# chalharu/rust-compression

Measured on AMD Instinct MI355X. Metric: BZip2 level-9 encode MB/s (input bytes, HBM-resident in and out: the kernels' rate; value_end_to_end is host buffer to host buffer at the C ABI), higher is better.
Workload: dtype u8/u32

## Files before the change

### rust-compression_amd/csrc/bzgpu.h

```cpp
#pragma once
#include <hip/hip_runtime.h>
#include <stdint.h>
#include <stddef.h>

namespace bzgpu {

typedef uint8_t u8;
typedef uint16_t u16;
typedef uint32_t u32;
typedef uint64_t u64;
typedef int64_t i64;

constexpr u32 kWave = 64;
constexpr u32 kMaxBlockLen = 900000;
constexpr u32 kSortTile = 8192;
constexpr u32 kSortThreads = 512;
constexpr u32 kTilesPerBlock = 110;
constexpr u32 kSlot = kTilesPerBlock * kSortTile;
constexpr u32 kPtSlot = kSlot / 8u * 10u;
constexpr u32 kPairWords = 65536u / 32u;
constexpr u32 kMaxBins = 2048;
constexpr u32 kPerK = 8;
constexpr u32 kGSize = 50;
constexpr u32 kMaxSelectors = 18002;
// ... 164 lines not shown
typedef u32 u32x4_t __attribute__((ext_vector_type(4)));
__device__ __forceinline__ void st_sc1_x4(u32 *p, uint4 v)
{
    const u32x4_t r = {v.x, v.y, v.z, v.w};
    asm volatile("global_store_dwordx4 %0, %1, off\n\ts_nop 1" : : "v"(p), "v"(r) : "memory");
}
__device__ __forceinline__ uint4 ld_sc1_x4(const u32 *p)
{
    u32x4_t r;
    asm volatile("global_load_dwordx4 %0, %1, off nt\n\ts_waitcnt vmcnt(0)" : "=v"(r) : "v"(p) : "memory");
    return make_uint4(r.x, r.y, r.z, r.w);
}

__device__ __forceinline__ void ld_sc1_x4_issue(const u32 *p, u32x4_t &r)
{
    asm volatile("global_load_dwordx4 %0, %1, off nt" : "=&v"(r) : "v"(p) : "memory");
}
__device__ __forceinline__ void ld_x4_wait_all() { asm volatile("s_waitcnt vmcnt(0)" : : : "memory"); }

constexpr u32 kCrcPoly = 0x04C11DB7u;

__host__ __device__ inline u32 gf_mulmod(u32 a, u32 b)
{
    u32 r = 0;
#pragma unroll 4
    for (int i = 31; i >= 0; --i) {
        r = (r << 1) ^ ((r & 0x80000000u) ? kCrcPoly : 0u);
        if ((b >> i) & 1u) r ^= a;
    }
    return r;
}

__device__ __forceinline__ u32 gf_xpow_bytes(u64 nbytes, const u32 *__restrict__ xp2)
{
    u32 r = 1u;
    for (u32 k = 0; nbytes; ++k, nbytes >>= 1)
        if (nbytes & 1u) r = gf_mulmod(r, xp2[k]);
    return r;
}

__device__ __forceinline__ u32 crc_bytes_raw(const u8 *__restrict__ p, u64 len, const u32 *s_tab)
{
    u32 crc = 0;
    for (u64 i = 0; i < len; ++i) crc = s_tab[(crc >> 24) ^ p[i]] ^ (crc << 8);
    return crc;
}


struct RleBuffers {
    i64 *tile_last;
    i64 *carry_in;
    u32 *tile_crc;
    u32 *tile_count;
    u16 *sub_off;
    i64 *sub_rs;
    u64 *tile_off;
    u64 *total;
    u64 *cut_result;
    u64 *scan_part;
    u32 *lb_ctl;
    u64 *lb_rs;
    u64 *lb_off;
};

struct CutPlan {
    u64 L;
    u64 g_base;
    u64 own_hi;
    u64 w_min;
    u64 j_lo, j_hi;
    u64 tb, t1;
    u64 t_last;
    u64 t_eval;
};
struct CutBuffers {
    u64 *step_t0;
    u32 *step_nt;
    u64 *step_w0;
    u32 *tab;
    u16 *comp;
};

struct BwtArgs {
    const u8 *rle;
    const BlockDesc *blocks;
    u32 nb;
    u32 tiles;
    u32 *SA, *R, *KA, *VA, *KB, *VB;
    u32 *tile_hist;
    u32 *bin_base;
    u32 *count;
    u32 *count2;
    u32 *tile_nf;
    u8 *flags;
    u64 *newbits;
    int *tile_last_old;
    int *tile_last_new;
    u32 *nonfinal;
    unsigned long long *active;
    u32 *maxnf;
    u32 *per_k, *per_shift;
    u32 *lin_p, *lin_sig;
    u32 *bin_cursor;
    u32 *pb_gate;
    u32 *loc_stats;
    u8 *L;
    u32 *orig_ptr;
    u8 *ptext;
    u32 *pair_bits;
    const u8 *sym_code;
    const u8 *keyinfo;
    u32 *gh_tiles;
    u32 *gbase;
    u32 pack_blocks;
    u64 *abits;
    u32 *tile_state;
    u32 *tickets;
    u32 *sort_err;
    u32 *epoch;
    u8 *per_aux;
    u32 per_keyshift;
    u32 per_wide;
    u32 per_links;
    u32 *fused_state;
    u32 *tile_state_all;
    u32 fused;
    size_t tile_state_bytes;
};
constexpr u32 kSortEpochs = 1024;

constexpr u32 kMtfStride = kSlot + 64;
struct MtfArgs {
    const BlockDesc *blocks;
    u32 nb;
    u32 tiles;
    const u8 *L;
    u32 heads;
    u32 dense_permille;
    u8 *H;
    u16 *headbits;
    u32 *hcount;
    u32 *tile_hcnt;
    u32 *tile_hbase;
    const u32 *inuse_bits;
    u8 *summ;
    u16 *summ_len;
    u8 *init_state;
    u8 *rank8;
    int *ztile_last;
    u32 *ztile_cnt;
    u32 *zstate;
    u32 *ztick;
    u32 fused_zle;
    u16 *mtf;
    u32 *mtf_freq;
    BlockOut *out;
};

constexpr u32 kLim = 17;
constexpr u32 kLmRow = 2 * kMaxAlpha + 4;
constexpr u32 kLmWords = 2 * kLim * kLmRow + 5 * kMaxAlpha + 64;
constexpr u32 kSelStride = kMaxSelectors + 14;
constexpr u32 kGboStride = kMaxSelectors + 2;
struct HuffArgs {
    const BlockDesc *blocks;
    u32 nb;
    const u16 *mtf;
    u32 mtf_stride;
    const u32 *mtf_freq;
    const u32 *inuse_bits;
    const u32 *crc;
    const u32 *orig_ptr;
    u8 *selector;
    u32 *code_len;
    u32 *group_bitoff;
    u32 *lm_scratch;
    u8 *glen;
    unsigned long long *pack;
    u32 *rfreq;
    u32 *hlm;
    u32 *pass_stats;
    u32 *stream;
    BlockOut *out;
    u32 *error_flag;
};

struct AsmBlock {
    u64 src_word;
    u64 bit_len;
    u64 dst_bit;
};
struct PackBlock {
    u64 src_word, dst_word, nwords;
};
struct RleBatchItem {
    u64 in_off;
    u64 len;
    u64 rle_off;
};
struct FrameItem {
    u64 first_word;
    u64 trailer_bit;
    u32 combined_crc;
    u32 pad;
};

constexpr int BZ_DEC_E_DATA = -1;
struct DecCand {
    u64 bitpos;
    u32 type;
    u32 pad;
};
struct DecBlockInfo {
    u64 end_bit;
    u32 status;
    u32 stored_crc;
    u32 orig_ptr;
    u32 randomised;
    u32 n_in_use;
    u32 nsym;
    u32 next_head;
    u32 next_bits;
    u8 seq2unseq[256];
};

constexpr u32 kDecSampleStep = 128;
constexpr u32 kDecSamples = kMaxBlockLen / kDecSampleStep + 3;
constexpr u32 kSegCap = 4 * kDecSampleStep;
constexpr u32 kDecSubs = kSlot / 64;
struct KernelProf;
struct DecArgs {
    u32 nb;
    u32 tiles, sub_wgs;
    u32 cw;
    const u32 *slot;
    const DecBlockInfo *info;
    const u16 *sym;
    const u32 *nblock_max;
    u8 *perm;
    u32 *chunk_emit;
    u32 *tt_len;
    u32 *err;
    u8 *L;
    u32 *T;
    u8 *X;
    u32 *samp_next, *samp_len, *samp_off;
    u32 *cycle_len;
    uint4 *sub_trans;
    u32 *sub_off;
    u8 *sub_state;
    u32 *work_ctr;
    uint4 *walk_meta;
    u8 *seg_buf;
    u32 *seg_cont;
    u32 *long_list;
    u32 *out_len;
    u32 *thist;
    u32 *tbase;
    u32 *crc;
};
void launch_dec_scan(hipStream_t st, const u8 *in, u64 nbytes, DecCand *cands, u32 cap, u32 *count);
void launch_dec_blocks(hipStream_t st, const u8 *in, u64 nbytes, const DecCand *cands, u32 ncand, DecBlockInfo *info,
                       u16 *sym, u8 *sel_scratch);
constexpr u32 kDecEntrySkip = 0xFFFFFFFFu;
struct DecEntry {
    u64 off, len;
    u32 first_cand, ncand;
};
enum : u32 { kChainOk = 0, kChainData = 1, kChainMagicFirst = 2, kChainMagic = 3 };
struct DecChainEntry {
    u32 verdict;
    u32 streams;
    u32 irregular;
    u32 ntrue;
};
struct DecChainCand {
    u32 is_true, max_len;
    u32 stored_crc, nsym;
};
void launch_dec_scan_batch(hipStream_t st, const u8 *in, u64 span0, u64 span_end, const DecEntry *ents, u32 nent,
                           DecCand *cands, u32 cap, u32 *count);
void launch_dec_blocks_batch(hipStream_t st, const u8 *in, const DecEntry *ents, const DecCand *cands, u32 ncand,
                             DecBlockInfo *info, u16 *sym, u8 *sel_scratch);
void launch_dec_chain_batch(hipStream_t st, const u8 *in, const DecEntry *ents, u32 e0, u32 ne, const DecCand *cands,
                            u32 cand0, const DecBlockInfo *info, DecChainEntry *out_ent, DecChainCand *out_cand);
void launch_dec_mtf(hipStream_t st, const DecArgs &a, KernelProf *prof, int *rec);
void launch_dec_gather_windows(hipStream_t st, const u8 *in, u64 nbytes, const u64 *bases, u32 nw, u8 *out);
void launch_dec_walks(hipStream_t st, const DecArgs &a, u32 walk_wgs, hipStream_t st2, hipEvent_t ev_a, hipEvent_t ev_b,
                      KernelProf *prof, int rec[4]);
void launch_dec_expand(hipStream_t st, const DecArgs &a, const u64 *out_base, u8 *out);
void launch_dec_crc(hipStream_t st, const DecArgs &a, const u64 *out_base, const u8 *out, u32 max_out_len,
                    const u32 *crc_tab, const u32 *xp2, const u32 *xp16);

enum KernelId {
    KID_RADIX_HIST = 0,
    KID_RADIX_SCAN,
    KID_RADIX_SCATTER,
    KID_GROUP_FLAGS,
    KID_GROUP_APPLY,
    KID_LAST_COLUMN,
    KID_RADIX_SCATTER_LB,
    KID_GHIST_TEXT,
    KID_GHIST_SCAN,
    KID_RANK_PLACE,
    KID_PHASE_B_LOCAL,
    KID_GROUP_REFINE,
// ... 82 lines not shown
```

### rust-compression_amd/csrc/engine.hip

```cpp
#include "engine_state.h"

#include <algorithm>
#include <chrono>
#include <cstdio>
#include <cstdlib>
#include <cstring>
#include <vector>

#define MAILCHK(st, ...)                                                             \
    do {                                                                             \
        const MailSeg mail_segs_[] = {__VA_ARGS__};                                  \
        if (mail_fetch((st), mail_segs_, (int)(sizeof(mail_segs_) / sizeof(mail_segs_[0]))) != 0) return BZ_E_UNEXPECTED; \
    } while (0)

static int span_begin(bz_gpu_engine *g, int stage, hipStream_t st = nullptr)
{
    bz_gpu_engine::Span s;
    s.stage = stage;
    s.st = st ? st : g->st;
    if (hipEventCreate(&s.a) != hipSuccess || hipEventCreate(&s.b) != hipSuccess) return -1;
    (void)hipEventRecord(s.a, s.st);
    g->spans.push_back(s);
    return (int)g->spans.size() - 1;
}
// ... 600 lines not shown
        *j_next = j0 + closed;
        return BZ_OK;
    }
    ++g->cut_stats[0];
    if (res[0] > max_blocks) return BZ_E_UNEXPECTED;
    sc.tb = std::min<u64>(start_in / kRleTile, t0);
    sc.start_in = start_in;
    sc.nb = (size_t)res[0];
    sc.pending = true;
    sc.image_done = true;
    sc.span = -1;
    *n_blocks = sc.nb;
    *next_in = sc.nb || is_last ? res[1] : start_in;
    *s_next = res[3];
    *j_next = res[4];
    sp.want_halo_total = D;
    return BZ_OK;
}
static int slab_spec_finish(bz_gpu_engine *g, SlabSpec &sp, SlabCuts &sc)
{
    if (!sc.pending) return BZ_OK;
    if (!sp.image_done) return slab_image(g, sc);
    const RleBuffers rb = rle_buffers(g);
    const u64 t0 = g->slab_t0;
    sc.span = span_begin(g, 0);
    g->h_halo_total = sp.want_halo_total;
    if (sc.tb < t0) {
        launch_rle_scan(g->st, g->d_in, g->n_in, sc.tb, t0, sc.start_in, g->crc_tab.as<u32>(), g->xp16.as<u32>(), rb);
        launch_rle_count(g->st, g->d_in, g->n_in, sc.tb, t0, sc.start_in, -1, rb, nullptr);
        launch_rle_prefix(g->st, sc.tb, t0, rb, false);
        HIPCHK(hipMemcpyAsync(&g->h_halo_total, rb.total, 8, hipMemcpyDeviceToHost, g->st));
        image_launch(g, g->st, sc.tb, t0, sc.start_in, rb, g->rle.as<u8>() + sp.halo_cap - sp.want_halo_total);
    }
    HIPCHK(hipStreamWaitEvent(g->st, g->ev_aux, 0));
    return slab_image(g, sc);
}

extern "C" int bz_gpu_partition_slab_finish(bz_gpu_engine *g, uint64_t start_in, int is_last, size_t *n_blocks,
                                            uint64_t *next_in, int *tail_block)
{
    if (!g) return BZ_E_PARAM;
    SlabCuts sc;
    const int rc = slab_cuts(g, start_in, is_last, true, sc, n_blocks, next_in, tail_block);
    if (rc != BZ_OK) {
        if (sc.span >= 0) { span_end(g, sc.span); spans_collect(g); }
        return rc;
    }
    return slab_image(g, sc);
}

extern "C" int bz_gpu_partition(bz_gpu_engine *g, int level, const void *d_in, size_t n, int mode,
                                size_t *n_blocks, size_t *consumed, int *tail_block)
{
    if (!g || level < 1 || level > 9) return BZ_E_PARAM;
    if (n_blocks) *n_blocks = 0;
    if (consumed) *consumed = 0;
    if (tail_block) *tail_block = 0;
    const u64 ntiles = (n + kRleTile - 1) / kRleTile;
    int64_t last = -1;
    int rc = bz_gpu_partition_slab_begin(g, level, d_in, n, 0, ntiles, &last);
    if (rc != BZ_OK || n == 0) return rc;
    if ((rc = bz_gpu_partition_slab_count(g, -1)) != BZ_OK) return rc;
    uint64_t next = 0;
    rc = bz_gpu_partition_slab_finish(g, 0, mode == BZ_ACTION_RUN ? 0 : 1, n_blocks, &next, tail_block);
    if (consumed) *consumed = (size_t)next;
    return rc;
}

static BwtArgs make_bwt_args(bz_gpu_engine *g, u32 nb)
{
    BwtArgs x;
    x.rle = g->rle.as<u8>();
    x.blocks = g->lblocks.as<BlockDesc>();
    x.nb = nb;
    x.tiles = kTilesPerBlock;
    x.SA = g->SA.as<u32>();
    x.R = g->R.as<u32>();
    x.KA = g->KA.as<u32>();
    x.VA = g->VA.as<u32>();
    x.KB = g->KB.as<u32>();
    x.VB = g->VB.as<u32>();
    x.tile_hist = g->tile_hist.as<u32>();
    x.count = g->count.as<u32>();
    x.count2 = g->count2.as<u32>();
    x.tile_nf = g->tile_nf.as<u32>();
    x.bin_base = g->bin_base.as<u32>();
    x.flags = g->flags.as<u8>();
    x.newbits = g->newbits.as<u64>();
    x.tile_last_old = g->tlo.as<int>();
    x.tile_last_new = g->tln.as<int>();
    x.nonfinal = g->nonfinal.as<u32>();
    x.active = g->active.as<unsigned long long>();
    x.maxnf = reinterpret_cast<u32 *>(g->active.as<unsigned long long>() + 64);
    x.per_k = g->per_k.as<u32>();
    x.per_shift = g->per_shift.as<u32>();
    x.lin_p = g->lin_p.as<u32>();
    x.lin_sig = g->lin_sig.as<u32>();
    x.bin_cursor = g->bin_cursor.as<u32>();
    x.pb_gate = g->pb_gate.as<u32>();
    x.loc_stats = g->pb_gate.as<u32>() + g->ws_blocks;
    x.L = g->L.as<u8>();
    x.orig_ptr = g->orig_ptr.as<u32>();
    x.ptext = g->ptext.as<u8>();
    x.pair_bits = pair_keys_wanted() ? g->pair_bits.as<u32>() : nullptr;
    x.sym_code = g->sym_code.as<u8>();
    x.keyinfo = g->keyinfo.as<u8>();
    x.gh_tiles = g->gh_tiles.as<u32>();
    x.gbase = g->gbase.as<u32>();
    x.abits = g->abits.as<u64>();
    x.pack_blocks = 0;
    x.tile_state = g->tile_state.as<u32>();
    x.tickets = g->tickets.as<u32>();
    x.sort_err = g->tickets.p ? g->tickets.as<u32>() + (size_t)kSortEpochs * 8 : nullptr;
    x.epoch = &g->sort_epoch;
    x.fused_state = g->fused_state;
    x.tile_state_all = g->tile_state.as<u32>();
    x.tile_state_bytes = g->tile_state.cap;
    x.fused = fused_wanted() ? 1u : 0u;
    static const u32 want_links = (getenv("BZ_LINK_ROUND") && atoi(getenv("BZ_LINK_ROUND")) == 0) ? 0u : 1u;
    x.per_links = want_links;
    x.per_keyshift = 0;
    x.per_wide = 0;
    x.per_aux = g->mtf.as<u8>();
    return x;
}

static MtfArgs make_mtf_args(bz_gpu_engine *g, u32 nb)
{
    MtfArgs ma;
    ma.blocks = g->lblocks.as<BlockDesc>();
    ma.nb = nb;
    ma.tiles = kTilesPerBlock;
    ma.L = g->L.as<u8>();
    ma.inuse_bits = g->inuse_bits.as<u32>();
    ma.summ = g->summ.as<u8>();
    ma.summ_len = g->summ_len.as<u16>();
    ma.init_state = g->init_state.as<u8>();
    ma.rank8 = g->rank8.as<u8>();
    static const bool want_heads = !(getenv("BZ_MTF_HEADS") && atoi(getenv("BZ_MTF_HEADS")) == 0);
    ma.heads = want_heads ? 1u : 0u;
    static const u32 dense_permille = getenv("BZ_MTF_DENSE_PERMILLE") ? (u32)std::min(1000, std::max(0, atoi(getenv("BZ_MTF_DENSE_PERMILLE")))) : 750u;
    ma.dense_permille = dense_permille;
    ma.H = g->mtf_heads_buf.as<u8>();
    ma.headbits = g->headbits.as<u16>();
    ma.hcount = g->hcount.as<u32>();
    ma.tile_hcnt = g->tile_hcnt.as<u32>();
    ma.tile_hbase = g->tile_hbase.as<u32>();
    ma.ztile_last = g->ztile_last.as<int>();
    ma.ztile_cnt = g->ztile_cnt.as<u32>();
    ma.zstate = g->zstate.as<u32>();
    ma.ztick = g->ztick.as<u32>();
    static const bool want_fused_zle = !(getenv("BZ_FUSED_ZLE") && atoi(getenv("BZ_FUSED_ZLE")) == 0);
    ma.fused_zle = (want_fused_zle && !g->zle_fused_broken) ? 1u : 0u;
    ma.mtf = g->mtf.as<u16>();
    ma.mtf_freq = g->mtf_freq.as<u32>();
    ma.out = g->bout.as<BlockOut>();
    return ma;
}

static HuffArgs make_huff_args(bz_gpu_engine *g, u32 nb)
{
    HuffArgs ha;
    ha.blocks = g->lblocks.as<BlockDesc>();
    ha.nb = nb;
    ha.mtf = g->mtf.as<u16>();
    ha.mtf_stride = kMtfStride;
    ha.mtf_freq = g->mtf_freq.as<u32>();
    ha.inuse_bits = g->inuse_bits.as<u32>();
    ha.crc = g->lcrc.as<u32>();
    ha.orig_ptr = g->orig_ptr.as<u32>();
    ha.selector = g->selector.as<u8>();
    ha.code_len = g->code_len.as<u32>();
    ha.group_bitoff = g->group_bitoff.as<u32>();
    ha.lm_scratch = g->lm_scratch.as<u32>();
    ha.glen = g->hglen.as<u8>();
    ha.pack = g->hpack.as<unsigned long long>();
    ha.rfreq = g->hrfreq.as<u32>();
    ha.hlm = g->hlm.as<u32>();
    ha.pass_stats = g->debug_figures ? g->hpass.as<u32>() : nullptr;
    ha.stream = g->stream.as<u32>();
    ha.out = g->bout.as<BlockOut>();
    ha.error_flag = g->error_flag.as<u32>();
    return ha;
}

__global__ void k_test_bump(u32 *p, u32 n) { *p = (*p + 1u) % n; }
__global__ void k_test_swap(u8 *L, u32 n)
{
    for (u32 i = n / 2; i + 1 < n; ++i)
        if (L[i] != L[i + 1]) {
            const u8 t = L[i];
            L[i] = L[i + 1];
            L[i + 1] = t;
            return;
        }
}

static int sort_batch(bz_gpu_engine *g, const BwtArgs &ba, u32 max_n, u64 total_n, u64 *sorted, KernelProf *prof, u64 *round_active)
{
    launch_block_symbols(g->st, ba, g->inuse_bits.as<u32>(), const_cast<u8 *>(ba.sym_code), const_cast<u8 *>(ba.keyinfo));
    std::vector<u8> ki((size_t)ba.nb * 4);
    {
        const MailSeg sg = {ki.data(), ba.keyinfo, ki.size()};
        if (mail_fetch(g->st, &sg, 1) != 0) return -1;
    }
    bool wide = false;
    u32 min_chars = 8;
    u32 pack_blocks = 0;
    for (u32 i = 0; i < ba.nb; ++i) {
        if (ki[(size_t)i * 4 + 2] == 0 && ki[(size_t)i * 4] >= 8) wide = true;
        if (ki[(size_t)i * 4 + 1] < min_chars) min_chars = ki[(size_t)i * 4 + 1];
        if (ki[(size_t)i * 4 + 2] != 0 && ki[(size_t)i * 4] == 10) pack_blocks += 1;
    }
    BwtArgs bs = ba;
    bs.pack_blocks = pack_blocks;
    return run_bwt(g->st, bs, max_n, total_n, g->h_active, sorted, prof, round_active, wide, min_chars);
}

static int encode_batch(bz_gpu_engine *g, u32 nb, const std::vector<BlockDesc> &descs)
{
    hipEvent_t ev_fork = nullptr, ev_join = nullptr;
    const bool have_events = hipEventCreateWithFlags(&ev_fork, hipEventDisableTiming) == hipSuccess &&
                             hipEventCreateWithFlags(&ev_join, hipEventDisableTiming) == hipSuccess;
    u32 max_n = 0;
    u64 total_n = 0;
    for (u32 i = 0; i < nb; ++i) {
        max_n = std::max(max_n, descs[i].n);
        total_n += descs[i].n;
    }
    MtfArgs ma = make_mtf_args(g, nb);
    ma.tiles = std::min<u32>(kTilesPerBlock, std::max<u32>(1u, (max_n + kSortTile - 1u) / kSortTile));
    int sp = have_events ? span_begin(g, 1) : -1;
    u64 sorted = 0;
    const int rounds = have_events ? sort_batch(g, make_bwt_args(g, nb), max_n, total_n, &sorted, &g->prof, g->round_active) : -1;
    int rc = rounds < 0 ? BZ_E_UNEXPECTED : BZ_OK;
    if (rc == BZ_OK) {
        static const bool corrupt_test = getenv("BZ_TEST_CORRUPT") && atoi(getenv("BZ_TEST_CORRUPT")) != 0;
        if (corrupt_test && g->fused_state[0] == 0 && descs[0].n > 1)
            hipLaunchKernelGGL(k_test_bump, dim3(1), dim3(1), 0, g->st, g->orig_ptr.as<u32>(), descs[0].n);
        static const bool late_clear_test = getenv("BZ_TEST_LATE_CLEAR") && atoi(getenv("BZ_TEST_LATE_CLEAR")) != 0;
        if (late_clear_test && g->fused_state[0] == 0 && descs[0].n > 1)
            hipLaunchKernelGGL(k_test_swap, dim3(1), dim3(1), 0, g->st, g->L.as<u8>(), descs[0].n);
        span_end(g, sp);
        g->bwt_stats[0] = std::max<u64>(g->bwt_stats[0], (u64)rounds);
        g->bwt_stats[1] += sorted;
        g->bwt_stats[2] += 1;
        (void)hipEventRecord(ev_fork, g->st);
        (void)hipStreamWaitEvent(g->st2, ev_fork, 0);
        sp = span_begin(g, 2, g->st2);
        launch_mtf(g->st2, ma, &g->prof, total_n);
        span_end(g, sp);
        sp = span_begin(g, 3, g->st2);
        launch_huffman(g->st2, make_huff_args(g, nb));
        span_end(g, sp);
        (void)hipEventRecord(ev_join, g->st2);
        (void)hipStreamWaitEvent(g->st, ev_join, 0);
    }
    if (rc == BZ_OK && ma.fused_zle) {
        u32 tk[9] = {};
        const MailSeg sg = {tk, g->ztick.p, sizeof(tk)};
        if (mail_fetch(g->st, &sg, 1) != 0) {
            rc = BZ_E_UNEXPECTED;
        } else {
            static const bool fail_test = getenv("BZ_FUSED_ZLE_FAILTEST") != nullptr;
            bool bad = tk[8] != 0 || fail_test;
            for (u32 x = 0; x < 8; ++x)
                if (tk[x] != ma.tiles * (xcd_grid_y(nb) / 8u)) bad = true;
            if (bad) {
                fprintf(stderr, "bz2_mi355x: the one-launch ZLE stage misbehaved (tile tickets / look-back); stage redone with three kernels\n");
                g->zle_fused_broken = true;
                launch_mtf(g->st, make_mtf_args(g, nb));
                launch_huffman(g->st, make_huff_args(g, nb));
            }
        }
    }
    const bool idle = hipStreamSynchronize(g->st2) == hipSuccess;
    if ((hipStreamSynchronize(g->st) != hipSuccess || !idle) && rc == BZ_OK) rc = BZ_E_UNEXPECTED;
    if (ev_fork) (void)hipEventDestroy(ev_fork);
    if (ev_join) (void)hipEventDestroy(ev_join);
    return rc;
}

extern "C" size_t bz_gpu_block_count(const bz_gpu_engine *g) { return g ? g->h_blocks.size() : 0; }

static int encode_blocks_once(bz_gpu_engine *g, const std::vector<size_t> &mine, void *d_packed, size_t cap_words,
                              uint64_t *h_word_off, uint64_t *h_bit_len, uint32_t *h_crc, size_t *words_used)
{
    if (words_used) *words_used = 0;
    g->h_out.clear();
    g->h_out_nblock.clear();
    g->h_out_pass.clear();
    int rc = ensure_workspace(g, mine.size());
    if (rc != BZ_OK) return rc;
    HIPCHK(hipMemsetAsync(g->error_flag.p, 0, 4, g->st));

    u64 word_cursor = 0;
    std::vector<BlockDesc> descs;
    std::vector<u32> crcs;
    std::vector<BlockOut> outs;
    std::vector<PackBlock> pbs;
    for (size_t k0 = 0; k0 < mine.size(); k0 += g->ws_blocks) {
        const u32 nb = (u32)std::min(g->ws_blocks, mine.size() - k0);
        descs.resize(nb);
        crcs.resize(nb);
        for (u32 i = 0; i < nb; ++i) {
            descs[i] = g->h_blocks[mine[k0 + i]];
// ... 956 lines not shown
```

### rust-compression_amd/csrc/k_mtf.hip

```cpp
#include "bzgpu.h"
#include <cstdlib>

namespace bzgpu {

constexpr u32 kChunkWGs = (kMaxMtfChunks + 255) / 256;
constexpr u32 kMtfSmallAlpha = 96;

__device__ __forceinline__ u32 popc8(const u32 *b)
{
    u32 c = 0;
#pragma unroll
    for (int i = 0; i < 8; ++i) c += __popc(b[i]);
    return c;
}

__device__ __forceinline__ u32 block_excl_sum(u32 v, u32 *sh , u32 &total)
{
    const u32 l = lane_id(), w = threadIdx.x >> 6;
    const u32 inc = wave_incl_sum(v);
    if (l == 63) sh[w] = inc;
    __syncthreads();
    u32 carry = 0, tot = 0;
    for (u32 k = 0; k < kSortThreads / 64; ++k) {
        if (k < w) carry += sh[k];
// ... 258 lines not shown
    const u32 nchunks = (n + kMtfChunk - 1) / kMtfChunk;
    const u32 c0 = blockIdx.x * kMtfGroup;
    if (c0 + 1u >= nchunks) return;
    const u32 alpha = popc8(a.inuse_bits + lb * 8);
    const size_t rep0 = (size_t)lb * kMaxMtfChunks;
    const bool act = l * 4u < alpha;
    const u32 g32 = act ? reinterpret_cast<const u32 *>(a.init_state + (rep0 + c0) * 256u)[l] : 0u;
    for (u32 k = 0; k < kMtfGroup / 4u; ++k) {
        const u32 c = c0 + 1u + k * 4u + wv;
        const bool live = c < nchunks && c < c0 + kMtfGroup;
        reinterpret_cast<u32 *>(s_state[wv])[l] = g32;
        const u32 m = live ? (u32)a.summ_len[rep0 + c - 1u] : 0u;
        const u32 w = (live && act) ? reinterpret_cast<const u32 *>(a.summ + (rep0 + c - 1u) * 256u)[l] : 0u;
        (void)mtf_apply_report(s_state[wv], alpha, m, w, s_new[wv], s_mark[wv], l);
        if (live && act) reinterpret_cast<u32 *>(a.init_state + (rep0 + c) * 256u)[l] = reinterpret_cast<u32 *>(s_state[wv])[l];
    }
}


constexpr u32 kMtfSmallPairs = kMtfSmallAlpha / 2;
constexpr u32 kMtfSubBlocks = 16;
typedef short short2_t __attribute__((ext_vector_type(2)));
__device__ __forceinline__ short2_t as_short2(u32 v)
{
    short2_t r;
    __builtin_memcpy(&r, &v, 4);
    return r;
}
template <u32 PAIRS, u32 LANES, u32 ALPHA_LO, u32 SUB = 1>
__global__ __launch_bounds__(LANES) void k_mtf_ranks_small(MtfArgs a)
{
    constexpr u32 CL = LANES / SUB;
    __shared__ u32 s_last[PAIRS * CL];
    __shared__ u8 s_code[256];
    const u32 lb = blockIdx.y;
    const u32 n = mtf_len(a, lb);
    const u32 chunk0 = blockIdx.x * CL;
    const u32 sub = threadIdx.x % SUB;
    if (chunk0 * kMtfChunk >= n) return;
    const u32 *bits = a.inuse_bits + lb * 8;
    const u32 alpha = popc8(bits);
    if (alpha > 2u * PAIRS || alpha <= ALPHA_LO) return;
    for (u32 v = threadIdx.x; v < 256u; v += LANES) {
        u32 before = 0;
        for (u32 q = 0; q < (v >> 5); ++q) before += __popc(bits[q]);
        before += __popc(bits[v >> 5] & ((1u << (v & 31u)) - 1u));
        s_code[v] = (u8)before;
    }
    __syncthreads();
    const u32 chunk = chunk0 + threadIdx.x / SUB;
    const u32 beg = chunk * kMtfChunk;
    if (beg >= n) return;
    const u32 end = (beg + kMtfChunk < n) ? beg + kMtfChunk : n;
    const u32 npairs = (alpha + 1u) >> 1;
    u32 *my = s_last + threadIdx.x / SUB;
    constexpr u32 kPB = 32;
    static_assert(PAIRS % (2u * kPB) == 0 || PAIRS <= kMtfSmallPairs, "the compare loop takes the table two blocks at a time");
    const u32 npairs16 = ((npairs + 2u * kPB - 1u) / (2u * kPB) * (2u * kPB)) < PAIRS ? ((npairs + 2u * kPB - 1u) / (2u * kPB) * (2u * kPB)) : PAIRS;
    for (u32 q = sub; q < (SUB > 1 ? PAIRS : npairs16); q += SUB) my[q * CL] = 0x80008000u;
    if (SUB > 1) {
        __builtin_amdgcn_fence(__ATOMIC_ACQ_REL, "workgroup");
        __builtin_amdgcn_wave_barrier();
    }
    if (sub == 0) {
        const u8 *st = a.init_state + ((size_t)lb * kMaxMtfChunks + chunk) * 256u;
        for (u32 q = 0; q < alpha; ++q) {
            const u32 c = s_code[st[q]];
            const u32 t = (u32)(0xFFFFu - q) & 0xFFFFu;
            u32 wd = my[(c >> 1) * CL];
            wd = (c & 1u) ? ((wd & 0x0000FFFFu) | (t << 16)) : ((wd & 0xFFFF0000u) | t);
            my[(c >> 1) * CL] = wd;
        }
    }
    if (SUB > 1) {
        __builtin_amdgcn_fence(__ATOMIC_ACQ_REL, "workgroup");
        __builtin_amdgcn_wave_barrier();
    }
    const u8 *L = mtf_seq(a, lb);
    u8 *R8 = a.rank8 + (size_t)lb * kSlot;
    for (u32 v4 = 0; v4 < kMtfChunk / 64u; ++v4) {
        if (beg + v4 * 64u >= end) break;
        uint4 q4[4];
#pragma unroll
        for (u32 u = 0; u < 4; ++u) {
            const u32 pl = beg + v4 * 64u + u * 16u;
            q4[u] = (pl < end) ? *reinterpret_cast<const uint4 *>(L + pl) : make_uint4(0, 0, 0, 0);
        }
#pragma unroll
      for (u32 u = 0; u < 4; ++u) {
        const u32 v = v4 * 4u + u;
        const u32 p0 = beg + v * 16u;
        if (p0 >= end) break;
        const u32 wv[4] = {q4[u].x, q4[u].y, q4[u].z, q4[u].w};
        u32 ov[4] = {0, 0, 0, 0};
#pragma unroll
        for (u32 k = 0; k < 16; ++k) {
            u32 rank = 0;
            if (p0 + k < end) {
                const u32 c = s_code[(wv[k >> 2] >> ((k & 3) * 8)) & 0xFFu];
                const u32 wc = my[(c >> 1) * CL];
                const u32 lsu = (c & 1u) ? (wc >> 16) : (wc & 0xFFFFu);
                const short2_t ls2 = as_short2(lsu | (lsu << 16));
                short2_t acc = {0, 0};
              if (SUB == 1 && PAIRS > kMtfSmallPairs) {
                u32 ra[kPB], rb[kPB];
#pragma unroll
                for (u32 e = 0; e < kPB; ++e) ra[e] = my[e * CL];
                for (u32 q = 0; q < npairs16; q += 2u * kPB) {
#pragma unroll
                    for (u32 e = 0; e < kPB; ++e) rb[e] = my[(q + kPB + e) * CL];
#pragma unroll
                    for (u32 e = 0; e < kPB; ++e) acc -= __builtin_elementwise_sub_sat(ls2, as_short2(ra[e])) >> (short2_t){15, 15};
                    const u32 qn = (q + 2u * kPB < npairs16) ? q + 2u * kPB : 0u;
#pragma unroll
                    for (u32 e = 0; e < kPB; ++e) ra[e] = my[(qn + e) * CL];
#pragma unroll
                    for (u32 e = 0; e < kPB; ++e) acc -= __builtin_elementwise_sub_sat(ls2, as_short2(rb[e])) >> (short2_t){15, 15};
                }
              } else if (SUB > 1) {
                constexpr u32 PER = PAIRS / SUB;
                u32 ra[PER];
#pragma unroll
                for (u32 e = 0; e < PER; ++e) ra[e] = my[(sub * PER + e) * CL];
#pragma unroll
                for (u32 e = 0; e < PER; ++e) acc -= __builtin_elementwise_sub_sat(ls2, as_short2(ra[e])) >> (short2_t){15, 15};
              } else
                for (u32 q = 0; q < npairs; ++q) {
                    const short2_t wd = as_short2(my[q * CL]);
                    const short2_t neg = __builtin_elementwise_sub_sat(ls2, wd) >> (short2_t){15, 15};
                    acc -= neg;
                }
                rank = (u32)(int)acc.x + (u32)(int)acc.y;
                if (SUB > 1) {
#pragma unroll
                    for (u32 d = 1; d < SUB; d <<= 1) rank += (u32)__shfl_xor((int)rank, (int)d, 64);
                }
                const u32 t = (v * 16u + k) & 0xFFFFu;
                if (sub == 0) my[(c >> 1) * CL] = (c & 1u) ? ((wc & 0x0000FFFFu) | (t << 16)) : ((wc & 0xFFFF0000u) | t);
            }
            ov[k >> 2] |= rank << ((k & 3) * 8);
        }
        if (sub == 0) *reinterpret_cast<uint4 *>(R8 + p0) = make_uint4(ov[0], ov[1], ov[2], ov[3]);
      }
    }
}

struct ZSeg {
    u8 r[16];
    u32 valid;
    u32 p0;
    int next_nonzero;
};

__device__ __forceinline__ void zload(const MtfArgs &a, u32 lb, u32 n, u32 tile, ZSeg &s)
{
    const u8 *__restrict__ R8 = a.rank8 + (size_t)lb * kSlot;
    s.p0 = tile * kSortTile + threadIdx.x * 16u;
    s.valid = s.p0 < n ? ((n - s.p0) < 16u ? (n - s.p0) : 16u) : 0u;
    if (mtf_collapsed(a, lb)) {
        __shared__ __attribute__((aligned(16))) u8 s_hr[kSortTile + 32];
        __shared__ u32 s_hs[kSortThreads / 64];
        const u16 *hbits = a.headbits + (((size_t)lb * kSlot) >> 4);
        const u32 hb = s.valid ? (u32)hbits[s.p0 >> 4] : 0u;
        const u32 hbase = a.tile_hbase[lb * kTilesPerBlock + tile];
        const u32 m = a.hcount[lb];
        const u32 a0 = hbase & ~15u;
        {
            const u32 off = a0 + threadIdx.x * 16u;
            if (off < m) *reinterpret_cast<uint4 *>(s_hr + threadIdx.x * 16u) = *reinterpret_cast<const uint4 *>(R8 + off);
            if (threadIdx.x == 0 && a0 + kSortTile < m)
                *reinterpret_cast<uint4 *>(s_hr + kSortTile) = *reinterpret_cast<const uint4 *>(R8 + a0 + kSortTile);
        }
        u32 total;
        u32 pos = (hbase - a0) + block_excl_sum((u32)__popc(hb), s_hs, total);
#pragma unroll
        for (int k = 0; k < 16; ++k) {
            const bool h = (hb >> k) & 1u;
            s.r[k] = h ? s_hr[pos] : (u8)0;
            pos += h ? 1u : 0u;
        }
        const u32 nx = s.p0 + s.valid;
        s.next_nonzero = (s.valid == 0u || nx >= n) ? 1 : (int)(hbits[nx >> 4] & 1u);
        return;
    }
    if (s.valid) {
        const uint4 q = *reinterpret_cast<const uint4 *>(R8 + s.p0);
        const u32 wv[4] = {q.x, q.y, q.z, q.w};
#pragma unroll
        for (int k = 0; k < 16; ++k) s.r[k] = (u8)(wv[k >> 2] >> ((k & 3) * 8));
        const u32 nx = s.p0 + s.valid;
        s.next_nonzero = (nx >= n) ? 1 : (R8[nx] != 0);
    } else {
        s.next_nonzero = 1;
    }
}

__device__ __forceinline__ int block_excl_max_int(int v, int *sh )
{
    const u32 l = lane_id(), w = threadIdx.x >> 6;
    const int inc = wave_incl_max32(v);
    if (l == 63) sh[w] = inc;
    __syncthreads();
    int carry = -1;
    for (u32 k = 0; k < w; ++k) carry = sh[k] > carry ? sh[k] : carry;
    const int prev = __shfl_up(inc, 1, 64);
    const int ex = (l == 0) ? -1 : prev;
    __syncthreads();
    return ex > carry ? ex : carry;
}

__global__ __launch_bounds__(kSortThreads) void k_zle_last(MtfArgs a)
{
    __shared__ int s_last;
    const u32 lb = blockIdx.y, tile = blockIdx.x;
    const u32 n = a.blocks[lb].n;
    if (tile * kSortTile >= n) return;
    if (threadIdx.x == 0) s_last = -1;
    __syncthreads();
    ZSeg s;
    zload(a, lb, n, tile, s);
    int last = -1;
#pragma unroll
    for (u32 k = 0; k < 16; ++k)
        if (k < s.valid && s.r[k]) last = (int)(s.p0 + k);
#pragma unroll
    for (u32 dd = 32; dd >= 1; dd >>= 1) {
        const int o = __shfl_xor(last, dd, 64);
        last = o > last ? o : last;
    }
    if (lane_id() == 0 && last >= 0) atomicMax(&s_last, last);
    __syncthreads();
    if (threadIdx.x == 0) a.ztile_last[lb * kTilesPerBlock + tile] = s_last;
}

__device__ __forceinline__ u32 run_digits(u32 z) { return 31u - (u32)__clz(z + 1u); }

template <bool WRITE>
__global__ __launch_bounds__(kSortThreads) void k_zle_emit(MtfArgs a)
{
    __shared__ int s_mi[16];
    __shared__ u32 s_su[16];
    __shared__ u32 s_freq[kMaxAlpha + 2];
    __shared__ int s_carry;
    __shared__ u32 s_base;
    __shared__ u16 s_out[WRITE ? kSortTile + 64 : 1];
    const u32 lb = blockIdx.y, tile = blockIdx.x;
    const u32 n = a.blocks[lb].n;
    if (tile * kSortTile >= n) return;
    if (threadIdx.x == 0) {
        int c = -1;
        for (int t = (int)tile - 1; t >= 0 && c < 0; --t) c = a.ztile_last[lb * kTilesPerBlock + t];
        s_carry = c;
        if (WRITE) {
            u32 b = 0;
            for (u32 t = 0; t < tile; ++t) b += a.ztile_cnt[lb * kTilesPerBlock + t];
            s_base = b;
        }
    }
    if (WRITE)
        for (u32 i = threadIdx.x; i < kMaxAlpha + 2; i += kSortThreads) s_freq[i] = 0;
    __syncthreads();
    ZSeg s;
    zload(a, lb, n, tile, s);
    int last = -1;
#pragma unroll
    for (u32 k = 0; k < 16; ++k)
        if (k < s.valid && s.r[k]) last = (int)(s.p0 + k);
    int lnz = block_excl_max_int(last, s_mi);
    lnz = lnz > s_carry ? lnz : s_carry;
    u32 cnt = 0;
    {
        int ln = lnz;
#pragma unroll
        for (u32 k = 0; k < 16; ++k) {
            if (k < s.valid) {
                const u32 p = s.p0 + k;
                if (s.r[k]) {
                    ln = (int)p;
                    cnt += 1;
                } else {
                    const bool run_end = (k + 1 < s.valid) ? (s.r[(k + 1) & 15] != 0) : (s.next_nonzero != 0);
                    if (run_end) cnt += run_digits((u32)((int)p - ln));
                }
            }
        }
    }
    u32 total;
    u32 off = block_excl_sum(cnt, s_su, total);
    if (!WRITE) {
        if (threadIdx.x == 0) a.ztile_cnt[lb * kTilesPerBlock + tile] = total;
        return;
    }
    u16 *out = s_out + off;
    u32 hot0 = 0, hot1 = 0, hot2 = 0, hot3 = 0;
    {
        int ln = lnz;
#pragma unroll
        for (u32 k = 0; k < 16; ++k) {
            if (k < s.valid) {
                const u32 p = s.p0 + k;
                if (s.r[k]) {
                    ln = (int)p;
                    const u32 sym = (u32)s.r[k] + 1u;
                    *out++ = (u16)sym;
                    if (sym == 2u) ++hot2;
                    else if (sym == 3u) ++hot3;
                    else atomicAdd(&s_freq[sym], 1u);
                } else {
                    const bool run_end = (k + 1 < s.valid) ? (s.r[(k + 1) & 15] != 0) : (s.next_nonzero != 0);
                    if (run_end) {
                        u32 zc = (u32)((int)p - ln) + 1u;
                        while (zc > 1u) {
                            const u32 run = zc & 1u;
                            *out++ = (u16)run;
                            hot0 += run ^ 1u;
                            hot1 += run;
                            zc >>= 1;
                        }
                    }
                }
            }
        }
    }
    hot0 = wave_sum(hot0);
    hot1 = wave_sum(hot1);
    hot2 = wave_sum(hot2);
    hot3 = wave_sum(hot3);
    if ((threadIdx.x & 63u) == 0) {
        if (hot0) atomicAdd(&s_freq[0], hot0);
        if (hot1) atomicAdd(&s_freq[1], hot1);
        if (hot2) atomicAdd(&s_freq[2], hot2);
        if (hot3) atomicAdd(&s_freq[3], hot3);
    }
    __syncthreads();
    {
        u16 *dst = a.mtf + (size_t)lb * kMtfStride + s_base;
        for (u32 i = threadIdx.x; i < total; i += kSortThreads) dst[i] = s_out[i];
    }
    const bool last_tile = (tile + 1) * kSortTile >= n;
    if (last_tile && threadIdx.x == 0) {
        const u32 alpha_in = popc8(a.inuse_bits + lb * 8);
        const u32 eob = alpha_in + 1u;
        a.mtf[(size_t)lb * kMtfStride + s_base + total] = (u16)eob;
        atomicAdd(&s_freq[eob], 1u);
        a.out[lb].mtf_count = s_base + total + 1u;
        a.out[lb].in_use_count = alpha_in;
    }
    __syncthreads();
    for (u32 i = threadIdx.x; i < kMaxAlpha; i += kSortThreads)
        if (s_freq[i]) atomicAdd(&a.mtf_freq[(size_t)lb * kMaxAlpha + i], s_freq[i]);
}

__global__ __launch_bounds__(kSortThreads) void k_zle_fused(MtfArgs a)
{
    __shared__ int s_mi[16];
    __shared__ u32 s_su[16];
    __shared__ u32 s_freq[kMaxAlpha + 2];
    __shared__ int s_carry;
    __shared__ u32 s_base, s_ticket;
    __shared__ u16 s_out[kSortTile + 64];
    const u32 xcd = (u32)__builtin_amdgcn_s_getreg(20 | (3 << 11)) & 7u;
    const u32 my_tiles = a.tiles * ((a.nb + 7u - xcd) / 8u);
    if (threadIdx.x == 0) s_ticket = atomicAdd(&a.ztick[xcd], 1u);
    __syncthreads();
    const u32 slot = s_ticket;
    if (slot >= my_tiles) return;
    const u32 b8 = slot / a.tiles;
    const u32 tile = slot - b8 * a.tiles;
    const u32 lb = b8 * 8u + xcd;
    const u32 n = a.blocks[lb].n;
    if (tile * kSortTile >= n) return;
    for (u32 i = threadIdx.x; i < kMaxAlpha + 2; i += kSortThreads) s_freq[i] = 0;
    ZSeg s;
    zload(a, lb, n, tile, s);
    int last = -1;
#pragma unroll
    for (u32 k = 0; k < 16; ++k)
        if (k < s.valid && s.r[k]) last = (int)(s.p0 + k);
    int lnz = block_excl_max_int(last, s_mi);
    u32 *mystate = a.zstate + ((size_t)lb * kTilesPerBlock + tile) * 4u;
    u32 w_last = 0;
    if (threadIdx.x == 0) {
        int tl = -1;
        for (u32 k = 0; k < kSortThreads / 64; ++k) tl = s_mi[k] > tl ? s_mi[k] : tl;
        const u32 vl = tl >= 0 ? (u32)tl : kLbValMask;
        st_sc1_x4(mystate, make_uint4((tile ? kLbAgg : kLbIncl) | vl, 0u, 0u, 0u));
        int c = -1;
        if (tile) {
            u32 spins = 0;
            for (u32 p = tile; p > 0 && c < 0;) {
                --p;
                const u32 *src = a.zstate + ((size_t)lb * kTilesPerBlock + p) * 4u;
                uint4 v = ld_sc1_x4(src);
                while ((v.x & kLbFlagMask) == 0u) {
                    if (lb_give_up(spins, a.ztick + 8, kLbSpinMax >> 3)) {
                        atomicExch(a.ztick + 8, 1u);
                        v = make_uint4(kLbIncl, 0u, 0u, 0u);
                        break;
                    }
                    __builtin_amdgcn_s_sleep(2);
                    v = ld_sc1_x4(src);
                }
                const u32 x = v.x & kLbValMask;
                if (x != kLbValMask) c = (int)x;
                else if ((v.x & kLbFlagMask) == kLbIncl) break;
            }
        }
        w_last = kLbIncl | (tl >= 0 ? (u32)tl : (c >= 0 ? (u32)c : kLbValMask));
        if (tile) st_sc1_x4(mystate, make_uint4(w_last, 0u, 0u, 0u));
        s_carry = c;
    }
    __syncthreads();
    lnz = lnz > s_carry ? lnz : s_carry;
    u32 cnt = 0;
    {
        int ln = lnz;
#pragma unroll
        for (u32 k = 0; k < 16; ++k) {
            if (k < s.valid) {
                const u32 p = s.p0 + k;
                if (s.r[k]) {
                    ln = (int)p;
                    cnt += 1;
                } else {
                    const bool run_end = (k + 1 < s.valid) ? (s.r[(k + 1) & 15] != 0) : (s.next_nonzero != 0);
                    if (run_end) cnt += run_digits((u32)((int)p - ln));
                }
            }
        }
    }
    u32 total;
    const u32 off = block_excl_sum(cnt, s_su, total);
    if (threadIdx.x == 0) st_sc1_x4(mystate, make_uint4(w_last, (tile ? kLbAgg : kLbIncl) | total, 0u, 0u));
    u16 *out = s_out + off;
    u32 hot0 = 0, hot1 = 0, hot2 = 0, hot3 = 0;
    {
        int ln = lnz;
#pragma unroll
        for (u32 k = 0; k < 16; ++k) {
            if (k < s.valid) {
                const u32 p = s.p0 + k;
                if (s.r[k]) {
                    ln = (int)p;
                    const u32 sym = (u32)s.r[k] + 1u;
                    *out++ = (u16)sym;
                    if (sym == 2u) ++hot2;
                    else if (sym == 3u) ++hot3;
                    else atomicAdd(&s_freq[sym], 1u);
                } else {
                    const bool run_end = (k + 1 < s.valid) ? (s.r[(k + 1) & 15] != 0) : (s.next_nonzero != 0);
                    if (run_end) {
                        u32 zc = (u32)((int)p - ln) + 1u;
                        while (zc > 1u) {
                            const u32 run = zc & 1u;
                            *out++ = (u16)run;
                            hot0 += run ^ 1u;
                            hot1 += run;
                            zc >>= 1;
                        }
                    }
                }
            }
        }
    }
    hot0 = wave_sum(hot0);
    hot1 = wave_sum(hot1);
    hot2 = wave_sum(hot2);
    hot3 = wave_sum(hot3);
    if ((threadIdx.x & 63u) == 0) {
        if (hot0) atomicAdd(&s_freq[0], hot0);
        if (hot1) atomicAdd(&s_freq[1], hot1);
        if (hot2) atomicAdd(&s_freq[2], hot2);
        if (hot3) atomicAdd(&s_freq[3], hot3);
    }
    if (threadIdx.x == 0) {
        u32 base = 0;
        if (tile) {
            u32 spins = 0;
            for (u32 p = tile; p > 0;) {
                --p;
                const u32 *src = a.zstate + ((size_t)lb * kTilesPerBlock + p) * 4u;
                uint4 v = ld_sc1_x4(src);
                while ((v.y & kLbFlagMask) == 0u) {
                    if (lb_give_up(spins, a.ztick + 8, kLbSpinMax >> 3)) {
                        atomicExch(a.ztick + 8, 1u);
                        v = make_uint4(0u, kLbIncl, 0u, 0u);
                        break;
                    }
                    __builtin_amdgcn_s_sleep(2);
                    v = ld_sc1_x4(src);
                }
                base += v.y & kLbValMask;
                if ((v.y & kLbFlagMask) == kLbIncl) break;
            }
            st_sc1_x4(mystate, make_uint4(w_last, kLbIncl | ((base + total) & kLbValMask), 0u, 0u));
        }
        s_base = base;
    }
    __syncthreads();
    {
        u16 *dst = a.mtf + (size_t)lb * kMtfStride + s_base;
        for (u32 i = threadIdx.x; i < total; i += kSortThreads) dst[i] = s_out[i];
    }
    const bool last_tile = (tile + 1) * kSortTile >= n;
    if (last_tile && threadIdx.x == 0) {
        const u32 alpha_in = popc8(a.inuse_bits + lb * 8);
        const u32 eob = alpha_in + 1u;
        a.mtf[(size_t)lb * kMtfStride + s_base + total] = (u16)eob;
        atomicAdd(&s_freq[eob], 1u);
        a.out[lb].mtf_count = s_base + total + 1u;
        a.out[lb].in_use_count = alpha_in;
    }
    __syncthreads();
    for (u32 i = threadIdx.x; i < kMaxAlpha; i += kSortThreads)
        if (s_freq[i]) atomicAdd(&a.mtf_freq[(size_t)lb * kMaxAlpha + i], s_freq[i]);
}

void launch_mtf(hipStream_t st, const MtfArgs &a, KernelProf *prof, u64 total_n)
{
    (void)hipMemsetAsync(a.mtf_freq, 0, (size_t)a.nb * kMaxAlpha * sizeof(u32), st);
    if (a.heads) {
        const int pi = prof ? prof->begin(st, KID_MTF_HEADS, 2u * total_n + total_n / 2u) : -1;
        hipLaunchKernelGGL(k_mtf_heads_mark, dim3(a.tiles, a.nb), dim3(kSortThreads), 0, st, a);
        hipLaunchKernelGGL(k_mtf_heads_pack, dim3(a.tiles, a.nb), dim3(kSortThreads), 0, st, a);
        if (prof) prof->end(st, pi);
    }
    hipLaunchKernelGGL(k_mtf_summaries, dim3(kChunkWGs, a.nb), dim3(256), 0, st, a);
    hipLaunchKernelGGL(k_mtf_merge_groups, dim3(kMtfGroups, a.nb), dim3(64), 0, st, a);
    hipLaunchKernelGGL(k_mtf_group_starts, dim3(a.nb), dim3(64), 0, st, a);
    hipLaunchKernelGGL(k_mtf_chunk_starts, dim3(kMtfGroups, a.nb), dim3(256), 0, st, a);
    if (a.nb <= kMtfSubBlocks) {
        hipLaunchKernelGGL((k_mtf_ranks_small<kMtfSmallPairs, 256, 0, 8>), dim3((kMaxMtfChunks + 31) / 32, a.nb), dim3(256), 0, st, a);
        hipLaunchKernelGGL((k_mtf_ranks_small<128, 128, kMtfSmallAlpha, 8>), dim3((kMaxMtfChunks + 15) / 16, a.nb), dim3(128), 0, st, a);
    } else {
        hipLaunchKernelGGL((k_mtf_ranks_small<kMtfSmallPairs, 256, 0>), dim3(kChunkWGs, a.nb), dim3(256), 0, st, a);
        hipLaunchKernelGGL((k_mtf_ranks_small<128, 128, kMtfSmallAlpha>), dim3((kMaxMtfChunks + 127) / 128, a.nb), dim3(128), 0, st, a);
    }
    if (a.fused_zle) {
        (void)hipMemsetAsync(a.zstate, 0, (size_t)a.nb * kTilesPerBlock * 16, st);
        (void)hipMemsetAsync(a.ztick, 0, 64, st);
        hipLaunchKernelGGL(k_zle_fused, dim3(a.tiles, xcd_grid_y(a.nb)), dim3(kSortThreads), 0, st, a);
        return;
    }
    const dim3 grid(a.tiles, a.nb);
    hipLaunchKernelGGL(k_zle_last, grid, dim3(kSortThreads), 0, st, a);
    hipLaunchKernelGGL((k_zle_emit<false>), grid, dim3(kSortThreads), 0, st, a);
    hipLaunchKernelGGL((k_zle_emit<true>), grid, dim3(kSortThreads), 0, st, a);
}

}
```

Baseline: 15030.

## Drive fused zero-run encoding from compacted head positions for collapsed MTF blocks

For blocks whose MTF output is stored in collapsed form (head bits plus packed nonzero ranks), the fused ZLE kernel no longer expands every tile into 16 dense ranks per thread. Instead it scatters the head positions into shared memory and has each thread walk a contiguous slice of them. Zero-run digits and symbols are emitted directly from the gaps between positions. The goal is to cut the per-position work and the register-heavy dense expansion when most positions are zero. The cost is an extra shared-memory position array and another barrier, plus load imbalance across threads. The path is on by default and can be disabled with BZ_ZLE_HEADS=0.

```diff
diff --git a/rust-compression_amd/csrc/bzgpu.h b/rust-compression_amd/csrc/bzgpu.h
--- a/rust-compression_amd/csrc/bzgpu.h
+++ b/rust-compression_amd/csrc/bzgpu.h
@@ -340,6 +340,7 @@
     u32 *zstate;
     u32 *ztick;
     u32 fused_zle;
+    u32 zle_heads;
     u16 *mtf;
     u32 *mtf_freq;
     BlockOut *out;
diff --git a/rust-compression_amd/csrc/engine.hip b/rust-compression_amd/csrc/engine.hip
--- a/rust-compression_amd/csrc/engine.hip
+++ b/rust-compression_amd/csrc/engine.hip
@@ -776,6 +776,8 @@
     ma.ztick = g->ztick.as<u32>();
     static const bool want_fused_zle = !(getenv("BZ_FUSED_ZLE") && atoi(getenv("BZ_FUSED_ZLE")) == 0);
     ma.fused_zle = (want_fused_zle && !g->zle_fused_broken) ? 1u : 0u;
+    static const bool want_zle_heads = !(getenv("BZ_ZLE_HEADS") && atoi(getenv("BZ_ZLE_HEADS")) == 0);
+    ma.zle_heads = want_zle_heads ? 1u : 0u;
     ma.mtf = g->mtf.as<u16>();
     ma.mtf_freq = g->mtf_freq.as<u32>();
     ma.out = g->bout.as<BlockOut>();
diff --git a/rust-compression_amd/csrc/k_mtf.hip b/rust-compression_amd/csrc/k_mtf.hip
--- a/rust-compression_amd/csrc/k_mtf.hip
+++ b/rust-compression_amd/csrc/k_mtf.hip
@@ -434,37 +434,48 @@
     int next_nonzero;
 };
 
-__device__ __forceinline__ void zload(const MtfArgs &a, u32 lb, u32 n, u32 tile, ZSeg &s)
-{
+__device__ __forceinline__ const u8 *zload_heads(const MtfArgs &a, u32 lb, u32 n, u32 tile, u32 &hb, u32 &first, u32 &H)
+{
+    __shared__ __attribute__((aligned(16))) u8 s_hr[kSortTile + 32];
+    __shared__ u32 s_hs[kSortThreads / 64];
     const u8 *__restrict__ R8 = a.rank8 + (size_t)lb * kSlot;
+    const u32 p0 = tile * kSortTile + threadIdx.x * 16u;
+    hb = p0 < n ? (u32)a.headbits[(((size_t)lb * kSlot) >> 4) + (p0 >> 4)] : 0u;
+    const u32 hbase = a.tile_hbase[lb * kTilesPerBlock + tile];
+    const u32 m = a.hcount[lb];
+    const u32 a0 = hbase & ~15u;
+    const u32 off = a0 + threadIdx.x * 16u;
+    if (off < m) *reinterpret_cast<uint4 *>(s_hr + threadIdx.x * 16u) = *reinterpret_cast<const uint4 *>(R8 + off);
+    if (threadIdx.x == 0 && a0 + kSortTile < m)
+        *reinterpret_cast<uint4 *>(s_hr + kSortTile) = *reinterpret_cast<const uint4 *>(R8 + a0 + kSortTile);
+    first = block_excl_sum((u32)__popc(hb), s_hs, H);
+    return s_hr + (hbase - a0);
+}
+
+__device__ __forceinline__ void zseg_bounds(u32 n, u32 tile, ZSeg &s)
+{
     s.p0 = tile * kSortTile + threadIdx.x * 16u;
     s.valid = s.p0 < n ? ((n - s.p0) < 16u ? (n - s.p0) : 16u) : 0u;
-    if (mtf_collapsed(a, lb)) {
-        __shared__ __attribute__((aligned(16))) u8 s_hr[kSortTile + 32];
-        __shared__ u32 s_hs[kSortThreads / 64];
-        const u16 *hbits = a.headbits + (((size_t)lb * kSlot) >> 4);
-        const u32 hb = s.valid ? (u32)hbits[s.p0 >> 4] : 0u;
-        const u32 hbase = a.tile_hbase[lb * kTilesPerBlock + tile];
-        const u32 m = a.hcount[lb];
-        const u32 a0 = hbase & ~15u;
-        {
-            const u32 off = a0 + threadIdx.x * 16u;
-            if (off < m) *reinterpret_cast<uint4 *>(s_hr + threadIdx.x * 16u) = *reinterpret_cast<const uint4 *>(R8 + off);
-            if (threadIdx.x == 0 && a0 + kSortTile < m)
-                *reinterpret_cast<uint4 *>(s_hr + kSortTile) = *reinterpret_cast<const uint4 *>(R8 + a0 + kSortTile);
-        }
-        u32 total;
-        u32 pos = (hbase - a0) + block_excl_sum((u32)__popc(hb), s_hs, total);
-#pragma unroll
-        for (int k = 0; k < 16; ++k) {
-            const bool h = (hb >> k) & 1u;
-            s.r[k] = h ? s_hr[pos] : (u8)0;
-            pos += h ? 1u : 0u;
-        }
-        const u32 nx = s.p0 + s.valid;
-        s.next_nonzero = (s.valid == 0u || nx >= n) ? 1 : (int)(hbits[nx >> 4] & 1u);
-        return;
-    }
+}
+
+__device__ __forceinline__ void zseg_heads(const MtfArgs &a, u32 lb, u32 n, u32 tile, u32 hb, u32 pos, const u8 *hr, ZSeg &s)
+{
+    const u16 *hbits = a.headbits + (((size_t)lb * kSlot) >> 4);
+    zseg_bounds(n, tile, s);
+#pragma unroll
+    for (int k = 0; k < 16; ++k) {
+        const bool h = (hb >> k) & 1u;
+        s.r[k] = h ? hr[pos] : (u8)0;
+        pos += h ? 1u : 0u;
+    }
+    const u32 nx = s.p0 + s.valid;
+    s.next_nonzero = (s.valid == 0u || nx >= n) ? 1 : (int)(hbits[nx >> 4] & 1u);
+}
+
+__device__ __forceinline__ void zseg_positions(const MtfArgs &a, u32 lb, u32 n, u32 tile, ZSeg &s)
+{
+    const u8 *__restrict__ R8 = a.rank8 + (size_t)lb * kSlot;
+    zseg_bounds(n, tile, s);
     if (s.valid) {
         const uint4 q = *reinterpret_cast<const uint4 *>(R8 + s.p0);
         const u32 wv[4] = {q.x, q.y, q.z, q.w};
@@ -474,6 +485,17 @@
         s.next_nonzero = (nx >= n) ? 1 : (R8[nx] != 0);
     } else {
         s.next_nonzero = 1;
+    }
+}
+
+__device__ __forceinline__ void zload(const MtfArgs &a, u32 lb, u32 n, u32 tile, ZSeg &s)
+{
+    if (mtf_collapsed(a, lb)) {
+        u32 hb, first, total;
+        const u8 *hr = zload_heads(a, lb, n, tile, hb, first, total);
+        zseg_heads(a, lb, n, tile, hb, first, hr, s);
+    } else {
+        zseg_positions(a, lb, n, tile, s);
     }
 }
 
@@ -633,6 +655,36 @@
         if (s_freq[i]) atomicAdd(&a.mtf_freq[(size_t)lb * kMaxAlpha + i], s_freq[i]);
 }
 
+__device__ __forceinline__ int zle_look_back_last(const MtfArgs &a, u32 lb, u32 tile, u32 *mystate, int tl, u32 &w_last)
+{
+    const u32 vl = tl >= 0 ? (u32)tl : kLbValMask;
+    st_sc1_x4(mystate, make_uint4((tile ? kLbAgg : kLbIncl) | vl, 0u, 0u, 0u));
+    int c = -1;
+    if (tile) {
+        u32 spins = 0;
+        for (u32 p = tile; p > 0 && c < 0;) {
+            --p;
+            const u32 *src = a.zstate + ((size_t)lb * kTilesPerBlock + p) * 4u;
+            uint4 v = ld_sc1_x4(src);
+            while ((v.x & kLbFlagMask) == 0u) {
+                if (lb_give_up(spins, a.ztick + 8, kLbSpinMax >> 3)) {
+                    atomicExch(a.ztick + 8, 1u);
+                    v = make_uint4(kLbIncl, 0u, 0u, 0u);
+                    break;
+                }
+                __builtin_amdgcn_s_sleep(2);
+                v = ld_sc1_x4(src);
+            }
+            const u32 x = v.x & kLbValMask;
+            if (x != kLbValMask) c = (int)x;
+            else if ((v.x & kLbFlagMask) == kLbIncl) break;
+        }
+    }
+    w_last = kLbIncl | (tl >= 0 ? (u32)tl : (c >= 0 ? (u32)c : kLbValMask));
+    if (tile) st_sc1_x4(mystate, make_uint4(w_last, 0u, 0u, 0u));
+    return c;
+}
+
 __global__ __launch_bounds__(kSortThreads) void k_zle_fused(MtfArgs a)
 {
     __shared__ int s_mi[16];
@@ -641,6 +693,7 @@
     __shared__ int s_carry;
     __shared__ u32 s_base, s_ticket;
     __shared__ u16 s_out[kSortTile + 64];
+    __shared__ u16 s_pos[kSortTile + 2];
     const u32 xcd = (u32)__builtin_amdgcn_s_getreg(20 | (3 << 11)) & 7u;
     const u32 my_tiles = a.tiles * ((a.nb + 7u - xcd) / 8u);
     if (threadIdx.x == 0) s_ticket = atomicAdd(&a.ztick[xcd], 1u);
@@ -653,70 +706,95 @@
     const u32 n = a.blocks[lb].n;
     if (tile * kSortTile >= n) return;
     for (u32 i = threadIdx.x; i < kMaxAlpha + 2; i += kSortThreads) s_freq[i] = 0;
-    ZSeg s;
-    zload(a, lb, n, tile, s);
-    int last = -1;
-#pragma unroll
-    for (u32 k = 0; k < 16; ++k)
-        if (k < s.valid && s.r[k]) last = (int)(s.p0 + k);
-    int lnz = block_excl_max_int(last, s_mi);
     u32 *mystate = a.zstate + ((size_t)lb * kTilesPerBlock + tile) * 4u;
     u32 w_last = 0;
-    if (threadIdx.x == 0) {
-        int tl = -1;
-        for (u32 k = 0; k < kSortThreads / 64; ++k) tl = s_mi[k] > tl ? s_mi[k] : tl;
-        const u32 vl = tl >= 0 ? (u32)tl : kLbValMask;
-        st_sc1_x4(mystate, make_uint4((tile ? kLbAgg : kLbIncl) | vl, 0u, 0u, 0u));
-        int c = -1;
-        if (tile) {
-            u32 spins = 0;
-            for (u32 p = tile; p > 0 && c < 0;) {
-                --p;
-                const u32 *src = a.zstate + ((size_t)lb * kTilesPerBlock + p) * 4u;
-                uint4 v = ld_sc1_x4(src);
-                while ((v.x & kLbFlagMask) == 0u) {
-                    if (lb_give_up(spins, a.ztick + 8, kLbSpinMax >> 3)) {
-                        atomicExch(a.ztick + 8, 1u);
-                        v = make_uint4(kLbIncl, 0u, 0u, 0u);
-                        break;
+    u32 total;
+    u32 hot0 = 0, hot1 = 0, hot2 = 0, hot3 = 0;
+    if (a.zle_heads && mtf_collapsed(a, lb)) {
+        const u32 tbase = tile * kSortTile;
+        const bool tail = tbase + kSortTile >= n;
+        u32 hb, first, H;
+        const u8 *hr = zload_heads(a, lb, n, tile, hb, first, H);
+        for (u32 j = first; hb; ++j, hb &= hb - 1u) s_pos[j] = (u16)(threadIdx.x * 16u + (u32)__builtin_ctz(hb));
+        if (tail && threadIdx.x == 0) s_pos[H] = (u16)(n - tbase);
+        __syncthreads();
+        const bool z0 = tile == 0u && hr[0] == 0;
+        int carry = -1;
+        if (threadIdx.x == 0) {
+            const int tl = (H == 0u || (H == 1u && z0)) ? -1 : (int)(tbase + s_pos[H - 1u]);
+            carry = zle_look_back_last(a, lb, tile, mystate, tl, w_last) - (int)tbase;
+        }
+        const u32 hv = H + (tail ? 1u : 0u);
+        const u32 per = ((hv + kSortThreads - 1u) / kSortThreads) | 1u;
+        const u32 i0 = threadIdx.x * per, i1 = i0 + per < hv ? i0 + per : hv;
+        const int prev0 = (i0 == 0u || (i0 == 1u && z0) || i0 >= hv) ? carry : (int)s_pos[i0 - 1u];
+        u32 cnt = 0;
+        {
+            int prev = prev0;
+            for (u32 i = i0; i < i1; ++i) {
+                const int p = (int)s_pos[i];
+                const bool sym = i < H && hr[i];
+                cnt += run_digits((u32)(p - prev - 1)) + (sym ? 1u : 0u);
+                prev = sym ? p : prev;
+            }
+        }
+        const u32 off = block_excl_sum(cnt, s_su, total);
+        if (threadIdx.x == 0) st_sc1_x4(mystate, make_uint4(w_last, (tile ? kLbAgg : kLbIncl) | total, 0u, 0u));
+        u16 *out = s_out + off;
+        int prev = prev0;
+        for (u32 i = i0; i < i1; ++i) {
+            const int p = (int)s_pos[i];
+            const u32 rank = i < H ? (u32)hr[i] : 0u;
+            for (u32 zc = (u32)(p - prev); zc > 1u; zc >>= 1) {
+                const u32 bit = zc & 1u;
+                *out++ = (u16)bit;
+                hot0 += bit ^ 1u;
+                hot1 += bit;
+            }
+            if (rank) {
+                const u32 sym = rank + 1u;
+                *out++ = (u16)sym;
+                if (sym == 2u) ++hot2;
+                else if (sym == 3u) ++hot3;
+                else atomicAdd(&s_freq[sym], 1u);
+            }
+            prev = rank ? p : prev;
+        }
+    } else {
+        ZSeg s;
+        zload(a, lb, n, tile, s);
+        int last = -1;
+#pragma unroll
+        for (u32 k = 0; k < 16; ++k)
+            if (k < s.valid && s.r[k]) last = (int)(s.p0 + k);
+        int lnz = block_excl_max_int(last, s_mi);
+        if (threadIdx.x == 0) {
+            int tl = -1;
+            for (u32 k = 0; k < kSortThreads / 64; ++k) tl = s_mi[k] > tl ? s_mi[k] : tl;
+            s_carry = zle_look_back_last(a, lb, tile, mystate, tl, w_last);
+        }
+        __syncthreads();
+        lnz = lnz > s_carry ? lnz : s_carry;
+        u32 cnt = 0;
+        {
+            int ln = lnz;
+#pragma unroll
+            for (u32 k = 0; k < 16; ++k) {
+                if (k < s.valid) {
+                    const u32 p = s.p0 + k;
+                    if (s.r[k]) {
+                        ln = (int)p;
+                        cnt += 1;
+                    } else {
+                        const bool run_end = (k + 1 < s.valid) ? (s.r[(k + 1) & 15] != 0) : (s.next_nonzero != 0);
+                        if (run_end) cnt += run_digits((u32)((int)p - ln));
                     }
-                    __builtin_amdgcn_s_sleep(2);
-                    v = ld_sc1_x4(src);
                 }
-                const u32 x = v.x & kLbValMask;
-                if (x != kLbValMask) c = (int)x;
-                else if ((v.x & kLbFlagMask) == kLbIncl) break;
-            }
-        }
-        w_last = kLbIncl | (tl >= 0 ? (u32)tl : (c >= 0 ? (u32)c : kLbValMask));
-        if (tile) st_sc1_x4(mystate, make_uint4(w_last, 0u, 0u, 0u));
-        s_carry = c;
-    }
-    __syncthreads();
-    lnz = lnz > s_carry ? lnz : s_carry;
-    u32 cnt = 0;
-    {
-        int ln = lnz;
-#pragma unroll
-        for (u32 k = 0; k < 16; ++k) {
-            if (k < s.valid) {
-                const u32 p = s.p0 + k;
-                if (s.r[k]) {
-                    ln = (int)p;
-                    cnt += 1;
-                } else {
-                    const bool run_end = (k + 1 < s.valid) ? (s.r[(k + 1) & 15] != 0) : (s.next_nonzero != 0);
-                    if (run_end) cnt += run_digits((u32)((int)p - ln));
-                }
-            }
-        }
-    }
-    u32 total;
-    const u32 off = block_excl_sum(cnt, s_su, total);
-    if (threadIdx.x == 0) st_sc1_x4(mystate, make_uint4(w_last, (tile ? kLbAgg : kLbIncl) | total, 0u, 0u));
-    u16 *out = s_out + off;
-    u32 hot0 = 0, hot1 = 0, hot2 = 0, hot3 = 0;
-    {
+            }
+        }
+        const u32 off = block_excl_sum(cnt, s_su, total);
+        if (threadIdx.x == 0) st_sc1_x4(mystate, make_uint4(w_last, (tile ? kLbAgg : kLbIncl) | total, 0u, 0u));
+        u16 *out = s_out + off;
         int ln = lnz;
 #pragma unroll
         for (u32 k = 0; k < 16; ++k) {
```

After: 15190, median of 6. +1.0%, better.
